# gotaku6629/CTC

Measured on AMD Instinct MI355X. Metric: ctc_samples_per_sec, higher is better.
Workload: dtype f32; 1 GPU; NoBlankCTC B=256 T=150 C=158 S<=20 fp32 (BASELINE configs[1]); variant=noblank, per_gpu_batch=256, global_batch=256, T=150, C=158, S=20, parallelism=dp1 (batch-sharded), launch=graph, graph_steps=50, step=fused loss+grad launch + scale_grad launch (loss.backward(), grad_out=1)

## Files before the change

### ctc_amd/build.py

```python
import os
import shutil
import subprocess
import sys

HERE = os.path.dirname(os.path.abspath(__file__))
CSRC = os.path.join(HERE, "csrc")
LIBDIR = os.path.join(HERE, "lib")
SO = os.path.join(LIBDIR, "libctc_amd.so")
SOURCES = ["api.hip", "noblank.hip", "binary.hip", "blank.hip", "decode.hip", "blank_align.hip", "targets.hip", "producer.hip"]
FLAGS = ["--offload-arch=gfx950", "-O3", "-std=c++17", "-fPIC", "-Wall", "-Wno-unused-function"]


def _hipcc():
    exe = shutil.which("hipcc") or "/opt/rocm/bin/hipcc"
    if not os.path.exists(exe):
        raise RuntimeError("hipcc not found: cannot build libctc_amd.so")
    return exe


def _stale():
    if not os.path.exists(SO):
        return True
    t = os.path.getmtime(SO)
    deps = [os.path.join(CSRC, f) for f in os.listdir(CSRC)] + \
           [os.path.join(HERE, "..", "include", "ctc_amd.h")]
    return any(os.path.getmtime(d) > t for d in deps)


def build(force=False, verbose=False, extra_flags=(), name=None):
    so = SO if name is None else os.path.join(LIBDIR, "libctc_amd_%s.so" % name)
    if name is None and any(f.startswith(("-DCTC_X_", "-DCTC_AMD_EXPERIMENTS", "-DCTC_AMD_FAULT_INJECT",
                                          "-DCTC_AMD_DIAGNOSTICS")) for f in extra_flags):
        raise RuntimeError("ctc_amd.build: experiment / diagnostics / fault-injection flags %s are refused for the "
                           "product library -- give the variant a name" % (list(extra_flags),))
    if name is None and not force and not _stale():
        return so
    os.makedirs(LIBDIR, exist_ok=True)
    objdir = os.path.join(LIBDIR, "obj" if name is None else "obj_" + name)
    os.makedirs(objdir, exist_ok=True)
    hipcc = _hipcc()
    procs = []
    for src in SOURCES:
        obj = os.path.join(objdir, src.replace(".hip", ".o"))
        cmd = [hipcc, *FLAGS, *extra_flags, "-c", os.path.join(CSRC, src), "-o", obj]
        if verbose:
            print(" ".join(cmd))
        procs.append((src, obj, subprocess.Popen(cmd, stdout=subprocess.PIPE, stderr=subprocess.STDOUT)))
    objs = []
    for src, obj, pr in procs:
        out, _ = pr.communicate()
        if pr.returncode != 0:
            raise RuntimeError("hipcc failed on %s:\n%s" % (src, out.decode()))
        if verbose and out:
            print(out.decode())
        objs.append(obj)
    subprocess.check_call([hipcc, "--offload-arch=gfx950", "-shared", "-fPIC", "-o", so + ".tmp", *objs])
    os.replace(so + ".tmp", so)
    return so


def _build_variant(name, flag, verbose):
    so = os.path.join(LIBDIR, "libctc_amd_%s.so" % name)
    if os.path.exists(so) and os.path.getmtime(so) >= os.path.getmtime(build()):
        return so
    return build(force=True, verbose=verbose, extra_flags=(flag,), name=name)


def build_diag(verbose=False):
    return _build_variant("diag", "-DCTC_AMD_DIAGNOSTICS", verbose)


def build_fault(verbose=False):
    return _build_variant("fault", "-DCTC_AMD_FAULT_INJECT", verbose)


def build_occupant():
    src = os.path.join(HERE, "..", "tools", "micro", "coresident.hip")
    so = os.path.join(LIBDIR, "libcoresident.so")
    if os.path.exists(so) and os.path.getmtime(so) >= os.path.getmtime(src):
        return so
    os.makedirs(LIBDIR, exist_ok=True)
    subprocess.check_call([_hipcc(), "--offload-arch=gfx950", "-O2", "-shared", "-fPIC", src, "-o", so + ".tmp"])
    os.replace(so + ".tmp", so)
    return so


HOST_EXT_DIR = os.path.join(LIBDIR, "ext")
HOST_EXT_SO = os.path.join(HOST_EXT_DIR, "ctc_amd_autograd_ext.so")


HOST_EXT_STAMP = os.path.join(HOST_EXT_DIR, "built_for_torch.txt")


def host_ext_is_current():
    import torch
    src = os.path.join(CSRC, "autograd_ext.cpp")
    if not (os.path.exists(HOST_EXT_SO) and os.path.exists(HOST_EXT_STAMP)):
        return False
    if os.path.getmtime(HOST_EXT_SO) < os.path.getmtime(src):
        return False
    return open(HOST_EXT_STAMP).read().strip() == torch.__version__


def build_host_ext(verbose=False):
    import torch
    src = os.path.join(CSRC, "autograd_ext.cpp")
    if host_ext_is_current():
        return HOST_EXT_SO
    from torch.utils import cpp_extension
    os.makedirs(HOST_EXT_DIR, exist_ok=True)
    cpp_extension.load(name="ctc_amd_autograd_ext", sources=[src], build_directory=HOST_EXT_DIR, extra_cflags=["-O2"],
                       with_cuda=False, verbose=verbose, is_python_module=False)
    with open(HOST_EXT_STAMP, "w") as f:
        f.write(torch.__version__)
    return HOST_EXT_SO


if __name__ == "__main__":
    if "--diag" in sys.argv:
        print(build_diag(verbose=True))
    else:
        print(build(force="--force" in sys.argv, verbose=True))
```

### ctc_amd/csrc/common.hpp

```cpp
#pragma once
#include <hip/hip_runtime.h>
#include <stdint.h>

#if !defined(CTC_AMD_EXPERIMENTS) &&                                                                            \
    (defined(CTC_X_NOSTATUS) || defined(CTC_X_NOREDUCE) || defined(CTC_X_NORETURN) || defined(CTC_X_NOCHAIN) || \
     defined(CTC_X_NOPRIO) || defined(CTC_X_NOREAD) || defined(CTC_X_NOWRITE) ||                                 \
     defined(CTC_X_WMASK) || defined(CTC_X_NOPROG) || defined(CTC_X_NORENORM) ||                                \
     defined(CTC_X_ROWDPP) || defined(CTC_X_SCALAR_STEP) || defined(CTC_X_NO_POOL_GATHER) || defined(CTC_X_FLOW_NO_GPRIO) || defined(CTC_X_FLOW_NOEXP) || defined(CTC_X_FLOW_NO_DELEGATE) || defined(CTC_X_FLOW_DELEGATE_OWN) || \
     defined(CTC_FLOW_TILE_WAVES))
#error "CTC_X_* experiment switches need -DCTC_AMD_EXPERIMENTS (A/B builds only, never the product library)"
#endif

namespace ctc {

constexpr int kWave = 64;
constexpr float kNeg = -10000000000000.0f;
constexpr float kInfeasible = 1.0e12f;

struct LaneStates { int K, SP; };
inline LaneStates lane_states(int S)
{
    int K = 1;
    while (K <= 4 && S > kWave * K) K *= 2;
    return {K, (S + K - 1) / K * K};
// ... 187 lines not shown
__device__ __forceinline__ float half_pick(float v, bool upper)
{
    const float lo = __builtin_bit_cast(float, __builtin_amdgcn_readlane(__builtin_bit_cast(int, v), 31));
    const float hi = __builtin_bit_cast(float, __builtin_amdgcn_readlane(__builtin_bit_cast(int, v), 63));
    return upper ? hi : lo;
}
__device__ __forceinline__ void halves_sum2(float &a, float &b, bool upper)
{
    asm volatile(CTC_REDUCE2_HALVES("v_add_f32_dpp") : "+v"(a), "+v"(b));
    a = half_pick(a, upper); b = half_pick(b, upper);
}
__device__ __forceinline__ void halves_max2(float &a, float &b, bool upper)
{
    asm volatile(CTC_REDUCE2_HALVES("v_max_f32_dpp") : "+v"(a), "+v"(b));
    a = half_pick(a, upper); b = half_pick(b, upper);
}

template <bool MAX>
__device__ __forceinline__ float group_reduce(float v, int G)
{
    v = MAX ? row16_max(v) : row16_sum(v);
    if (G >= 32) { const float o = __shfl_xor(v, 16, kWave); v = MAX ? fmaxf(v, o) : v + o; }
    if (G >= 64) { const float o = __shfl_xor(v, 32, kWave); v = MAX ? fmaxf(v, o) : v + o; }
    return v;
}

__device__ __forceinline__ float vmax(float a, float b)
{
    float r;
    asm("v_max_f32_e32 %0, %1, %2" : "=v"(r) : "v"(a), "v"(b));
    return r;
}

__device__ __forceinline__ float vmax3(float a, float b, float c)
{
    float r;
    asm("v_max3_f32 %0, %1, %2, %3" : "=v"(r) : "v"(a), "v"(b), "v"(c));
    return r;
}

constexpr float kLog2e = 1.4426950408889634f, kLn2 = 0.6931471805599453f;
__device__ __forceinline__ float fast_exp(float x) { return __builtin_amdgcn_exp2f(x * kLog2e); }
__device__ __forceinline__ float fast_log(float x) { return __builtin_amdgcn_logf(x) * kLn2; }

__device__ __forceinline__ float lse2(float a, float b)
{
    const float m = a > b ? a : b;
    const float t = __builtin_amdgcn_exp2f(-fabsf(a - b) * kLog2e);
    return __builtin_fmaf(__builtin_amdgcn_logf(1.0f + t), kLn2, m);
}

__device__ __forceinline__ int load_label(const void *p, int is64, int64_t i)
{
    return static_cast<const int32_t *>(p)[is64 ? 2 * i : i];
}

struct ScalarLengths {
    int64_t a, b;
    __device__ __forceinline__ ScalarLengths() : a(0), b(0) {}
    __device__ __forceinline__ ScalarLengths(const int64_t *pa, const int64_t *pb)
    {
        typedef const __attribute__((address_space(4))) int64_t const_i64;
        a = *(const_i64 *)(uintptr_t)pa;
        b = *(const_i64 *)(uintptr_t)pb;
    }
    __device__ __forceinline__ void get(int64_t &va, int64_t &vb) const
    {
        va = a;
        vb = b;
    }
};

__device__ __forceinline__ void bce_logs(float x, float &p, float &lp, float &lq)
{
    p = 1.0f / (1.0f + expf(-x));
    lp = fmaxf(logf(p), -100.0f);
    lq = fmaxf(logf(1.0f - p), -100.0f);
}

template <typename P>
__device__ __forceinline__ void stamp(const P &p, int slot)
{
    if (CTC_DIAG(p) >= 0 || CTC_DIAG(p) <= -100) return;
    if (blockIdx.x == 0 && wave_id() == -CTC_DIAG(p) - 1 && lane_id() == 0) {
        unsigned long long *o = reinterpret_cast<unsigned long long *>(p.counter) + 8 + 2 * slot;
        o[0] = __builtin_amdgcn_s_memtime();
        o[1] = __builtin_amdgcn_s_memrealtime();
    }
}

template <typename P>
__device__ __forceinline__ void stamp_setup(const P &p, int slot)
{
    if (CTC_DIAG(p) > -100 || CTC_DIAG(p) <= -200) return;
    if (blockIdx.x == 0 && wave_id() == -CTC_DIAG(p) - 100 && lane_id() == 0) {
        unsigned long long *o = reinterpret_cast<unsigned long long *>(p.counter) + 8 + 2 * slot;
        o[0] = __builtin_amdgcn_s_memtime();
        o[1] = __builtin_amdgcn_s_memrealtime();
    }
}

template <typename P>
__device__ __forceinline__ void stamp_mode(const P &p, int base, int slot)
{
    if (CTC_DIAG(p) > base || CTC_DIAG(p) <= base - 64) return;
    if (blockIdx.x == 0 && wave_id() == base - CTC_DIAG(p) && lane_id() == 0) {
        unsigned long long *o = reinterpret_cast<unsigned long long *>(p.counter) + 8 + 2 * (slot % 12);
        o[0] = __builtin_amdgcn_s_memtime();
        o[1] = __builtin_amdgcn_s_memrealtime();
    }
}

__device__ __forceinline__ void publish_value(float value, int b, float *nll)
{
    if (lane_id() == 0) __hip_atomic_store(&nll[b], value, __ATOMIC_RELAXED, __HIP_MEMORY_SCOPE_AGENT);
}
template <typename F>
__device__ __forceinline__ void ticket_and_reduce(int B, float *nll, float *loss, float loss_scale, unsigned *counter,
                                                  F per_sample)
{
    int last = 0;
    if (lane_id() == 0) {
        asm volatile("s_waitcnt vmcnt(0)" ::: "memory");
        unsigned ticket = __hip_atomic_fetch_add(counter, 1u, __ATOMIC_RELAXED, __HIP_MEMORY_SCOPE_AGENT);
        last = (ticket == (unsigned)(B - 1));
    }
    last = __builtin_amdgcn_readfirstlane(last);
    if (!last) return;
    float s = 0.f;
    for (int i = lane_id(); i < B; i += kWave)
        s += per_sample(__hip_atomic_load(&nll[i], __ATOMIC_RELAXED, __HIP_MEMORY_SCOPE_AGENT), i);
    s = wave_sum(s);
    if (lane_id() == 0) {
        loss[0] = s * loss_scale;
        __hip_atomic_store(counter, 0u, __ATOMIC_RELAXED, __HIP_MEMORY_SCOPE_AGENT);
        reset_arrivals(counter);
    }
}
template <typename F>
__device__ __forceinline__ void publish_and_reduce(float value, int b, int B, float *nll,
                                                   float *loss, float loss_scale,
                                                   unsigned *counter, F per_sample)
{
    publish_value(value, b, nll);
#ifndef CTC_X_NOREDUCE
    ticket_and_reduce(B, nll, loss, loss_scale, counter, per_sample);
#endif
}

constexpr int kAccIntBits = 13, kAccMaxB = 4095, kAccShards = 16;
__device__ __forceinline__ int acc_frac_bits(int B)
{
    return 40 - kAccIntBits - (B <= 1 ? 0 : 32 - __builtin_clz((unsigned)(B - 1)));
}
__host__ __device__ inline size_t acc_list_bytes(int B) { return 256 + (((size_t)4 * B + 255) & ~(size_t)255); }
__device__ __forceinline__ void publish_and_reduce_sum(float value, int b, int B, float *nll, float *loss,
                                                       float loss_scale, unsigned *counter)
{
    if (B > kAccMaxB) {
        publish_and_reduce(value, b, B, nll, loss, loss_scale, counter, [](float x, int) { return x; });
        return;
    }
    if (lane_id() != 0) return;
    unsigned long long *top = reinterpret_cast<unsigned long long *>(counter + 4);
    unsigned long long *shards = reinterpret_cast<unsigned long long *>(counter + 64);
    unsigned *nlist = counter + 6, *list = counter + 128;
    __hip_atomic_store(&nll[b], value, __ATOMIC_RELAXED, __HIP_MEMORY_SCOPE_AGENT);
// ... 38 lines not shown
```

### ctc_amd/csrc/noblank.hip

```cpp
#include <type_traits>

#include "lattice.hpp"
#include "launch.hpp"

namespace ctc {

struct NoblankParams {
    const float *x;
    int64_t st, sb;
    const void *lab;
    int lab64;
    const int64_t *in_len, *tgt_len;
    int T, B, C, S, SP;
    int stop;
    float loss_scale, grad_scale;
    float *nll, *loss, *grad;
    float *gamma;
    float *lattice;
    int64_t slab;
    unsigned *counter;
    int next_round;
    float ls_a, ls_b;
    int koff;
};
// ... 304 lines not shown
            const int t0 = base + w * kRows;
            for (int r = 0; r < kRows; r += per)
                if (t0 + r < Tlive)
                    posterior_row<true>(sm.al, sm.be, sm.em, sm.nxt, sm.dup, t0 + r + sub,
                                  r + sub < kRows && t0 + r + sub < Tlive, L, p.SP, G);
            if (CTC_DIAG(p) == 4) continue;
            stamp(p, 6);
            if (base == 0) {
                rows.grad(p, sm, b, t0, Tlive, first);
            } else {
                Rows<CHR> extra;
                extra.load(p, b, t0, Tlive);
                extra.grad(p, sm, b, t0, Tlive, first);
            }
        }
    } else {
        rows_grad_generic(p, sm, b, Tlive, L);
    }
    stamp(p, 7);
}

}

#include "noblank_pipe.hpp"
#include "noblank_xr.hpp"
#include "noblank_r16.hpp"
#ifdef CTC_AMD_DIAGNOSTICS
#include "noblank_km.hpp"
#endif

namespace ctc {

__global__ __launch_bounds__(256) void scale_grad_kernel(float *g, const float *go, size_t n)
{
    const float s = *go;
    if (s == 1.0f) return;
    const size_t stride = (size_t)gridDim.x * blockDim.x;
    size_t i = (size_t)blockIdx.x * blockDim.x + threadIdx.x;
    if ((reinterpret_cast<uintptr_t>(g) & 15) == 0) {
        float4 *g4 = reinterpret_cast<float4 *>(g);
        const size_t n4 = n / 4;
        for (size_t k = i; k < n4; k += stride) {
            float4 v = g4[k];
            v.x *= s; v.y *= s; v.z *= s; v.w *= s;
            g4[k] = v;
        }
        for (size_t k = n4 * 4 + i; k < n; k += stride) g[k] *= s;
    } else {
        for (size_t k = i; k < n; k += stride) g[k] *= s;
    }
}

template <typename E>
__global__ __launch_bounds__(256) void scale_grad_lowp_kernel(E *g, const float *go, size_t n)
{
    const float s = *go;
    if (s == 1.0f) return;
    const size_t stride = (size_t)gridDim.x * blockDim.x;
    const size_t i = (size_t)blockIdx.x * blockDim.x + threadIdx.x;
    size_t done = 0;
    if ((reinterpret_cast<uintptr_t>(g) & 7) == 0) {
        wt_u2 *g4 = reinterpret_cast<wt_u2 *>(g);
        const size_t n4 = n / 4;
        const f2_t s2 = {s, s};
        for (size_t k = i; k < n4; k += stride) {
            wt_u2 v = g4[k];
            v.x = r16_narrow2<E>(r16_widen2<E>(v.x) * s2);
            v.y = r16_narrow2<E>(r16_widen2<E>(v.y) * s2);
            g4[k] = v;
        }
        done = n4 * 4;
    }
    for (size_t k = done + i; k < n; k += stride) g[k] = (E)((float)g[k] * s);
}


struct NoblankSwitches {
    bool no_pipe, no_xr, no_r16, no_ps, km;
    bool nograd;
    int stop;
};
static const NoblankSwitches &noblank_switches()
{
    static const NoblankSwitches sw = {diag_env("CTC_AMD_NOPIPE") != 0, diag_env("CTC_AMD_NOXR") != 0,
                                       diag_env("CTC_AMD_NOR16") != 0,  diag_env("CTC_AMD_NOPS") != 0,
                                       diag_env("CTC_AMD_KM") != 0,     diag_env("CTC_AMD_DEBUG_NOGRAD") != 0,
                                       diag_env("CTC_AMD_DEBUG_STOP")};
    return sw;
}

static int noblank_params(NoblankParams &p, const void *x, int64_t stride_t, int64_t stride_b,
                          const void *labels, int labels_i64, const int64_t *in_len, const int64_t *tgt_len,
                          int T, int B, int C, int S, float loss_scale, float grad_scale,
                          float *nll, float *loss, void *grad, float *gamma, void *workspace, float label_smoothing,
                          const NoblankSwitches &sw)
{
    if (!x || !labels || !in_len || !tgt_len || !nll || !(loss || gamma) || !workspace) return CTC_AMD_ERR_BAD_ARGUMENT;
    if (T < 1 || B < 1 || C < 1 || S < 1) return CTC_AMD_ERR_BAD_ARGUMENT;
    const NoblankSizes z = noblank_sizes(T, C, S);
    char *ws = static_cast<char *>(workspace);
    p.x = static_cast<const float *>(x); p.st = stride_t; p.sb = stride_b;
    p.lab = labels; p.lab64 = labels_i64;
    p.in_len = in_len; p.tgt_len = tgt_len;
    p.T = T; p.B = B; p.C = C; p.S = S; p.SP = z.SP;
    p.stop = sw.stop;
    p.loss_scale = loss_scale; p.grad_scale = grad_scale;
    p.nll = nll; p.loss = gamma ? reinterpret_cast<float *>(ws + 32) : loss;
    p.grad = sw.nograd ? nullptr : static_cast<float *>(grad);
    p.gamma = gamma;
    p.counter = static_cast<unsigned *>(workspace);
    p.lattice = z.glb ? reinterpret_cast<float *>(ws + 256 + acc_list_bytes(B)) : nullptr;
    p.slab = z.glb ? (int64_t)noblank_lattice_floats(T, z.SP) : 0;
    p.next_round = 0; p.koff = 0;
    const bool smooth = label_smoothing >= 0.f;
    p.ls_b = smooth ? (1.f - label_smoothing) / (float)C : 0.f;
    p.ls_a = smooth ? label_smoothing - p.ls_b : 1.f;
    return 0;
}

struct NoblankQuery {
    int T, B, C, S;
    int dtype;
    int64_t st, sb;
    unsigned x_low, grad_low;
    bool want_grad, want_gamma, smooth;
    int cus;
    NoblankSwitches sw;
};
enum NoblankFamily { kNoblankUnsupported = 0, kNoblankR16, kNoblankKm, kNoblankXr, kNoblankPipelined, kNoblankFused };
struct NoblankPlan {
    int family;
    int n4, n2, nt, ps;
    int ch, dual;
    int K, glb;
    int grid;
    size_t lds;
    int next_round, koff;
};

static bool r16_takes(const NoblankQuery &q, const NoblankSizes &z, unsigned align, int &n4, int &n2)
{
    return z.K == 1 && q.T <= kPipeMaxT && q.C % 2 == 0 && q.st % 2 == 0 && q.sb % 2 == 0 && q.x_low % align == 0 &&
           q.grad_low % align == 0 && r16_shape(q.C, n4, n2) && z.SP <= 31 && r16_smem_bytes(q.T, z.SP, q.C) <= kMaxLds;
}

static NoblankPlan noblank_plan(const NoblankQuery &q)
{
    const NoblankSizes z = noblank_sizes(q.T, q.C, q.S);
    NoblankPlan pl = {};
    if (z.K > 4) return pl;
    const bool lowp = q.dtype != CTC_AMD_F32;
    const int esz = lowp ? 2 : 4, cus = q.cus;
    pl.grid = q.B;
    int n4 = 0, n2 = 0;
    const bool r16 = r16_takes(q, z, lowp ? 4 : 8, n4, n2);
    const bool r16_only = q.smooth || lowp;
    const bool fast = z.K == 1 && q.C <= 256 && q.T <= kPipeMaxT && !q.sw.no_pipe && !z.glb && !q.want_gamma;
    if (r16 && (q.want_gamma || lowp || (fast && !q.sw.no_r16))) {
        pl.n4 = n4; pl.n2 = n2;
        pl.lds = r16_smem_bytes(q.T, z.SP, q.C);
        if (q.want_gamma) { pl.family = kNoblankR16; return pl; }
        pl.nt = (size_t)2 * esz * q.T * q.B * q.C > ((size_t)230 << 20);
#ifdef CTC_AMD_DIAGNOSTICS
        const int koff = km_offset(q.T, q.S);
        if (q.sw.km && !lowp && km_smem_bytes(q.T, z.SP, q.C) <= kMaxLds && koff >= 0) {
            pl.family = kNoblankKm;
            pl.lds = km_smem_bytes(q.T, z.SP, q.C);
            pl.koff = koff;
            pl.next_round = (q.B > cus && (size_t)q.T * ((q.C * 4 + 127) / 128) <= (size_t)kKmWorkers * kWave) ? cus : 0;
            return pl;
        }
#endif
        pl.family = kNoblankR16;
        pl.next_round = (q.B > cus && (size_t)q.T * ((q.C * esz + 127) / 128) <= (size_t)kPipeWorkers * kWave) ? cus : 0;
        pl.ps = q.B > 2 * cus && cus > 0 && !q.sw.no_ps && q.want_grad && 4 * n4 + 2 * n2 <= 12;
        if (pl.ps) pl.grid = cus;
        return pl;
    }
    if (r16_only || (z.glb && z.smem > kMaxLds)) return NoblankPlan{};
    if (fast) {
        pl.ch = (q.C + kWave - 1) / kWave;
        pl.dual = q.B > cus && 2 * z.smem <= kMaxLds;
        const size_t xsmem = xr_smem_bytes(q.T, z.SP, q.C);
        const bool xr = !q.sw.no_xr && xsmem <= kMaxLds && (!pl.dual || 2 * xsmem <= kMaxLds);
        pl.family = xr ? kNoblankXr : kNoblankPipelined;
        pl.lds = xr ? xsmem : z.smem;
        return pl;
    }
    pl.family = kNoblankFused;
    pl.K = z.K; pl.glb = z.glb;
    pl.ch = q.C <= 256 && !z.glb ? (q.C + kWave - 1) / kWave : 0;
    pl.lds = z.smem;
    return pl;
}

template <int N, int... Ns, typename F>
static int with_constant(int n, F f)
{
    if constexpr (sizeof...(Ns) == 0) {
        return f(std::integral_constant<int, N>());
    } else {
        return n == N ? f(std::integral_constant<int, N>()) : with_constant<Ns...>(n, f);
    }
}
template <typename F>
static int with_row_chunks(int n4, int n2, F f)
{
    return with_constant<1, 2, 4, 5, 6, 8, 9, 10, 12, 13, 14, 16>(4 * n4 + n2, [&](auto k) {
        return f(std::integral_constant<int, decltype(k)::value / 4>(), std::integral_constant<int, decltype(k)::value % 4>());
    });
}

static int noblank_launch(const NoblankPlan &pl, int dtype, NoblankParams &p, hipStream_t s)
{
    const dim3 grid(pl.grid), block(kThreads);
    p.next_round = pl.next_round; p.koff = pl.koff;
    switch (pl.family) {
        case kNoblankR16:
            return with_row_chunks(pl.n4, pl.n2, [&](auto n4, auto n2) {
                return with_constant<0, 1>(pl.nt, [&](auto nt) {
                    return with_constant<CTC_AMD_BF16, CTC_AMD_F16, CTC_AMD_F32>(dtype, [&](auto dt) {
                        using E = std::conditional_t<decltype(dt)::value == CTC_AMD_BF16, __bf16,
                                                     std::conditional_t<decltype(dt)::value == CTC_AMD_F16, _Float16, float>>;
                        constexpr int A = decltype(n4)::value, Bq = decltype(n2)::value;
                        constexpr bool NT = decltype(nt)::value != 0;
                        if constexpr (4 * A + 2 * Bq <= 12)
                            if (pl.ps) return launch<noblank_r16_kernel<A, Bq, NT, true, E>>(grid, block, pl.lds, s, p);
                        return launch<noblank_r16_kernel<A, Bq, NT, false, E>>(grid, block, pl.lds, s, p);
                    });
                });
            });
#ifdef CTC_AMD_DIAGNOSTICS
        case kNoblankKm:
            return with_row_chunks(pl.n4, pl.n2, [&](auto n4, auto n2) {
                return with_constant<0, 1>(pl.nt, [&](auto nt) {
                    return launch<noblank_km_kernel<decltype(n4)::value, decltype(n2)::value, decltype(nt)::value != 0>>(
                        grid, block, pl.lds, s, p);
                });
            });
#endif
        case kNoblankXr:
        case kNoblankPipelined:
            return with_constant<1, 2, 3, 4>(pl.ch, [&](auto ch) {
                return with_constant<0, 1>(pl.dual, [&](auto dual) {
                    constexpr int CH = decltype(ch)::value;
                    constexpr bool DUAL = decltype(dual)::value != 0;
                    return pl.family == kNoblankXr ? launch<noblank_xr_kernel<CH, DUAL>>(grid, block, pl.lds, s, p)
                                                   : launch<noblank_pipelined_kernel<CH, DUAL>>(grid, block, pl.lds, s, p);
                });
            });
        case kNoblankFused:
            return with_constant<1, 2, 4>(pl.K, [&](auto k) {
                constexpr int K = decltype(k)::value;
                if (pl.glb) return launch<noblank_fused_kernel<K, 0, true>>(grid, block, pl.lds, s, p);
                return with_constant<1, 2, 3, 4, 0>(pl.ch, [&](auto ch) {
                    return launch<noblank_fused_kernel<K, decltype(ch)::value>>(grid, block, pl.lds, s, p);
                });
            });
        default: return CTC_AMD_ERR_UNSUPPORTED_SHAPE;
    }
}

static int noblank_run(const void *x, int64_t stride_t, int64_t stride_b,
                       const void *labels, int labels_i64,
                       const int64_t *in_len, const int64_t *tgt_len,
                       int T, int B, int C, int S,
                       float loss_scale, float grad_scale,
                       float *nll, float *loss, void *grad,
                       void *workspace, void *stream, float label_smoothing, int x_dtype = CTC_AMD_F32,
                       float *gamma = nullptr)
{
    const NoblankSwitches sw = gamma ? NoblankSwitches{} : noblank_switches();
    NoblankParams p;
    if (const int rc = noblank_params(p, x, stride_t, stride_b, labels, labels_i64, in_len, tgt_len, T, B, C, S, loss_scale,
                                      grad_scale, nll, loss, grad, gamma, workspace, label_smoothing, sw))
        return rc;
    const NoblankQuery q = {T, B, C, S, x_dtype, stride_t, stride_b,
                            (unsigned)(reinterpret_cast<uintptr_t>(x) & 15), (unsigned)(reinterpret_cast<uintptr_t>(grad) & 15),
                            p.grad != nullptr, gamma != nullptr, label_smoothing >= 0.f,
                            device_cus(),
                            sw};
    return noblank_launch(noblank_plan(q), x_dtype, p, static_cast<hipStream_t>(stream));
}

static dim3 scale_grad_grid(size_t n)
{
    size_t blocks = (n / 4 + 255) / 256;
    static const int cap = diag_env("CTC_AMD_SCALE_BLOCKS", 1024);
    if (blocks > (size_t)cap) blocks = cap;
    if (blocks < 1) blocks = 1;
    return dim3((unsigned)blocks);
}

}

using namespace ctc;

extern "C" int ctc_amd_noblank_loss_grad(const float *x, int64_t stride_t, int64_t stride_b,
                                         const void *labels, int labels_i64,
                                         const int64_t *in_len, const int64_t *tgt_len,
                                         int T, int B, int C, int S,
                                         float loss_scale, float grad_scale,
                                         float *nll, float *loss, float *grad,
                                         void *workspace, void *stream)
{
    return noblank_run(x, stride_t, stride_b, labels, labels_i64, in_len, tgt_len, T, B, C, S, loss_scale, grad_scale,
                       nll, loss, grad, workspace, stream, -1.f);
}

extern "C" int ctc_amd_noblank_smoothed_loss_grad(const float *x, int64_t stride_t, int64_t stride_b,
                                                  const void *labels, int labels_i64,
// ... 90 lines not shown
```

### ctc_amd/csrc/noblank_r16.hpp

```cpp
#pragma once

namespace ctc {

typedef float f2_t __attribute__((ext_vector_type(2)));

#define CTC_ROW16(OP)                                                                   \
    "s_nop 1\n\t" OP " %0, %0, %0 quad_perm:[1,0,3,2] row_mask:0xf bank_mask:0xf\n\t"   \
    "s_nop 1\n\t" OP " %0, %0, %0 quad_perm:[2,3,0,1] row_mask:0xf bank_mask:0xf\n\t"   \
    "s_nop 1\n\t" OP " %0, %0, %0 row_half_mirror row_mask:0xf bank_mask:0xf\n\t"       \
    "s_nop 1\n\t" OP " %0, %0, %0 row_mirror row_mask:0xf bank_mask:0xf\n\t"            \
    "s_nop 1"
__device__ __forceinline__ void row16_allmax(float &v) { asm volatile(CTC_ROW16("v_max_f32_dpp") : "+v"(v)); }
__device__ __forceinline__ void row16_allsum(float &v) { asm volatile(CTC_ROW16("v_add_f32_dpp") : "+v"(v)); }
__device__ __forceinline__ void row16_allmax(int &v) { asm volatile(CTC_ROW16("v_max_i32_dpp") : "+v"(v)); }

constexpr int kR16Pad = 2 * kPrefetch + 1;
#ifndef CTC_R16_BLOCK
#define CTC_R16_BLOCK 16
#endif
constexpr int kR16Block = CTC_R16_BLOCK;
__host__ __device__ inline int r16_pitch(int T)
{
    int tp = T + 2 * kR16Pad + 1;
    while ((tp & 3) != 2) ++tp;
    return tp;
}

__device__ __forceinline__ int r16_row(int T, int u, int g, int k)
{
    const int H = (T + 1) >> 1, idx = 2 * kPipeWorkers * g + 2 * u + (k >> 1);
    if ((k & 1) == 0) return idx < H ? idx : -1;
    return idx < T - H ? T - 1 - idx : -1;
}

struct R16Smem {
    int TP;
    cell_t *em, *al, *be;
    float *dummy, *stage, *cs;
    int *cnt, *lab, *occ, *done;
    __device__ R16Smem(float *base, int T, int SP, int RP)
    {
        TP = r16_pitch(T);
        cell_t *lat = reinterpret_cast<cell_t *>(base);
        em = lat + kR16Pad;
        al = em + (size_t)(SP + 1) * TP;
        be = al + (size_t)(SP + 1) * TP;
        dummy = reinterpret_cast<float *>(lat + (size_t)3 * (SP + 1) * TP);
        cnt = reinterpret_cast<int *>(dummy + 8);
        lab = cnt + 16;
        occ = lab + ((SP + 3) & ~3);
        cs = reinterpret_cast<float *>(occ + ((SP + 3) & ~3) + 4);
        done = reinterpret_cast<int *>(cs + 4 * kPipeWorkers);
        stage = cs + 64;
    }
};

static size_t r16_smem_bytes(int T, int SP, int C)
{
    const int RP = 32 * ((C + 31) / 32);
    return (size_t)3 * (SP + 1) * r16_pitch(T) * 8 + (8 + 16 + 2 * ((SP + 3) & ~3) + 4 + 64) * 4 +
           (size_t)kPipeWorkers * 4 * RP * 4;
}

template <bool FWD>
__device__ __forceinline__ cell_t r16_chain(const NoblankParams &p, const R16Smem &sm, int T, int Tb, int L, int SP, const int lane)
{
    constexpr int G = kPipeRows / 4;
    constexpr int D = FWD ? 1 : -1;
    const int lrow = lane < SP ? lane : SP;
    const cell_t *erow = sm.em + (size_t)lrow * sm.TP;
    cell_t *orow = (FWD ? sm.al : sm.be) + (size_t)lrow * sm.TP;
    typedef float pair_t __attribute__((ext_vector_type(4)));
    float m;
    int k;

    const int H = (T + 1) >> 1;
    const int pos0 = FWD ? 0 : T - Tb;
    const int own = FWD ? H : T - H;
    typedef const volatile __attribute__((address_space(3))) int lds_cvint;
    const int *cp = sm.cnt + (lane < kPipeWorkers ? lane : 0);
    int have = 0;
    bool starved = false;
    auto wait_upto = [&](int i_last) {
        const int q = pos0 + (i_last < Tb ? i_last : Tb - 1);
        int ng = q / (2 * kPipeWorkers) + 1;
        if (q >= own || ng > G) ng = G;
        if (ng <= have) return;
        const int need = lane < kPipeWorkers ? 4 * ng : 0;
        int spins = 0;
        while (__builtin_amdgcn_ballot_w64(*(lds_cvint *)cp < need) != 0) {
            if (++spins >= kSpinLimit) { starved = true; break; }
            __builtin_amdgcn_s_sleep(1);
        }
        lds_order();
        have = ng;
    };
#define CTC_R16_STEP_ASM(K, M, EM, EK, K2, T2, DPP)                                                  \
            "v_max_i32_dpp %[kk], " K ", " K " " DPP "\n\t"                                           \
            "v_add_u32 " K2 ", %[kk], " EK "\n\t"                                                     \
            "v_sub_u32 %[d1], " K ", %[kk]\n\t"                                                       \
            "v_sub_u32_dpp %[d2], " K ", %[kk] " DPP "\n\t"                                           \
            "v_ldexp_f32 %[d1], " EM ", %[d1]\n\t"                                                    \
            "v_ldexp_f32 %[d2], " EM ", %[d2]\n\t"                                                    \
// ... 296 lines not shown
        for (int k = 0; k < N2; ++k) o2[k] = *reinterpret_cast<const f2_t *>(trow + off2(k, i16));
#pragma unroll
        for (int j = 0; j < N4; ++j) {
            const f4_t o = o4[j];
            f2_t olo = {o.x, o.y}, ohi = {o.z, o.w};
            if (LS) { olo += cb2; ohi += cb2; }
            const f2_t xlo = {a[j].x, a[j].y}, xhi = {a[j].z, a[j].w};
            const f2_t vlo = __builtin_elementwise_fma(xlo, r2, olo), vhi = __builtin_elementwise_fma(xhi, r2, ohi);
            if (!(kLast4 && j == N4 - 1) || col_ok) {
                if constexpr (kLowp) {
                    const wt_u2 n = {r16_narrow2<E>(vlo), r16_narrow2<E>(vhi)};
                    grad_store<NT, wt_u2, 4>(reinterpret_cast<wt_u2 *>(g + off4(j, i16)), n);
                } else {
                    const f4_t v = {vlo.x, vlo.y, vhi.x, vhi.y};
                    grad_store<NT>(reinterpret_cast<f4_t *>(g + off4(j, i16)), v);
                }
            }
        }
#pragma unroll
        for (int k = 0; k < N2; ++k) {
            f2_t o = o2[k];
            if (LS) o += cb2;
            const f2_t v = __builtin_elementwise_fma(c[k], r2, o);
            if (k < N2 - 1 || col_ok) {
                if constexpr (kLowp) grad_store<NT, unsigned, 4>(reinterpret_cast<unsigned *>(g + off2(k, i16)), r16_narrow2<E>(v));
                else grad_store<NT>(reinterpret_cast<f2_t *>(g + off2(k, i16)), v);
            }
        }
    }
    __device__ __forceinline__ void touch() const
    {
        if constexpr (kLowp) {
#pragma unroll
            for (int j = 0; j < N4; ++j) asm volatile("" ::"v"(this->ra[j]));
#pragma unroll
            for (int k = 0; k < N2; ++k) asm volatile("" ::"v"(this->rc[k]));
        } else {
#pragma unroll
            for (int j = 0; j < N4; ++j) asm volatile("" ::"v"(a[j]));
#pragma unroll
            for (int k = 0; k < N2; ++k) asm volatile("" ::"v"(c[k]));
        }
    }
    template <bool NT>
    __device__ static __forceinline__ void store_zero(E *g, int i16, bool col_ok)
    {
        if constexpr (kLowp) {
            const wt_u2 z4 = {0u, 0u};
#pragma unroll
            for (int j = 0; j < N4; ++j)
                if (!(kLast4 && j == N4 - 1) || col_ok) grad_store<NT, wt_u2, 4>(reinterpret_cast<wt_u2 *>(g + off4(j, i16)), z4);
#pragma unroll
            for (int k = 0; k < N2; ++k)
                if (k < N2 - 1 || col_ok) grad_store<NT, unsigned, 4>(reinterpret_cast<unsigned *>(g + off2(k, i16)), 0u);
            return;
        }
        const f4_t z4 = {0.f, 0.f, 0.f, 0.f};
        const f2_t z2 = {0.f, 0.f};
#pragma unroll
        for (int j = 0; j < N4; ++j)
            if (!(kLast4 && j == N4 - 1) || col_ok) grad_store<NT>(reinterpret_cast<f4_t *>(g + off4(j, i16)), z4);
#pragma unroll
        for (int k = 0; k < N2; ++k)
            if (k < N2 - 1 || col_ok) grad_store<NT>(reinterpret_cast<f2_t *>(g + off2(k, i16)), z2);
    }
};

static bool r16_shape(int C, int &n4, int &n2)
{
    if (C < 2 || C > 256 || (C & 1)) return false;
    const int U = (C + 31) / 32;
    if (U & 1) { n4 = U / 2; n2 = 1; }
    else if ((C & 3) == 0) { n4 = U / 2; n2 = 0; }
    else { n4 = U / 2 - 1; n2 = 2; }
    return true;
}

template <typename E>
__device__ __forceinline__ const E *r16_xrow(const NoblankParams &p, int t, int b)
{
    return reinterpret_cast<const E *>(p.x) + (int64_t)t * p.st + (int64_t)b * p.sb;
}
template <int N4, int N2, bool NT, bool PS = false, typename E = float>
__global__ __launch_bounds__(kThreads, 4) void noblank_r16_kernel(NoblankParams p)
{
    extern __shared__ float4 smem_raw[];
    typedef R16Row<N4, N2, E> Row;
    constexpr int RP = Row::kCols;
    constexpr int G = kPipeRows / 4;
    const R16Smem sm(reinterpret_cast<float *>(smem_raw), p.T, p.SP, RP);
    const int tid = threadIdx.x, w = wave_id(), lane = lane_id();
    int vb = blockIdx.x;
    int b = xcd_sample(vb, p.B);
    if (tid == 64 * kChainB) note_arrival(p.counter, b);
    const int u = (w == 0 || w == kChainB) ? -1 : (w < kChainB ? w - 1 : w - 2);
    const int rho = lane >> 4, i16 = lane & 15;

    if (CTC_DIAG(p) == 1) return;
    stamp(p, 0);
    stamp_setup(p, 0);
    auto spread = [&](int which) {
        if (CTC_DIAG(p) != -50 || w != 1 || lane != 0) return;
        const int bid = blockIdx.x, nb = gridDim.x;
        const int slot = bid == 0 ? 0 : bid == nb / 2 ? 2 : bid == nb - 1 ? 4 : -1;
        if (slot < 0) return;
        unsigned long long *o = reinterpret_cast<unsigned long long *>(p.counter) + 8 + 2 * (slot + which);
        o[0] = __builtin_amdgcn_s_memtime();
        o[1] = __builtin_amdgcn_s_memrealtime();
    };
    spread(0);
    ScalarLengths len(p.in_len + b, p.tgt_len + b);
    int tv0[G];
    Row v[G];
#ifdef CTC_R16_NX
    constexpr int NX = PS ? CTC_R16_NX : 0;
#else
    constexpr int NX = PS ? (NT ? 2 : 3) : 0;
#endif
    Row nx[NX > 0 ? NX : 1];
    const bool col_ok = Row::off_last(i16) < p.C;
    const int c_last = col_ok ? Row::off_last(i16) : p.C - (Row::kLast4 ? 4 : 2);
    const int Hh = (p.T + 1) >> 1;
    bool grp[G];
#pragma unroll
    for (int g = 0; g < G; ++g) grp[g] = u >= 0 && 2 * kPipeWorkers * g + 2 * u < Hh;
    int klab = 0;
    if (PS && w == 0 && lane < p.S) klab = load_label(p.lab, p.lab64, (int64_t)b * p.S + lane);
    if (u >= 0) {
#pragma unroll
        for (int g = 0; g < G; ++g) {
            tv0[g] = r16_row(p.T, u, g, rho);
            if (g >= NX) v[g].load(r16_xrow<E>(p, tv0[g] >= 0 ? tv0[g] : 0, b), i16, c_last);
            else nx[g].load(r16_xrow<E>(p, tv0[g] >= 0 ? tv0[g] : 0, b), i16, c_last);
        }
        stamp_setup(p, 1);
        if (PS) {
#pragma unroll
            for (int g = 0; g < G; ++g) {
                if (g < NX) nx[g].touch();
                else v[g].touch();
            }
        }
    }
    const float ninf = -__builtin_inff();
    typedef const volatile __attribute__((address_space(3))) int lds_cvint;
    int Tb = 0, L = 0, bn = b, vbn = vb, klab_n = 0;
    bool more = false;
    ScalarLengths len_n;
    const cell_t zero = make_cell(0.f, 0);
    auto begin = [&](const bool chain_role) -> bool {
        int64_t Tb64, L64;
        len.get(Tb64, L64);
        stamp_setup(p, 2);
        const bool ok = L64 >= 1 && L64 <= p.S && Tb64 >= L64 && Tb64 <= p.T;
        Tb = ok ? (int)Tb64 : 0;
        L = ok ? (int)L64 : 0;
        vbn = vb + (int)gridDim.x;
        more = PS && vbn < p.B;
        bn = more ? xcd_sample(vbn, p.B) : b;
        if (PS) len_n = ScalarLengths(p.in_len + bn, p.tgt_len + bn);
        klab_n = 0;
        if (chain_role && w == 0) {
            int k = 0;
            if (lane < L) {
                k = (PS ? klab : load_label(p.lab, p.lab64, (int64_t)b * p.S + lane)) % p.C;
                if (k < 0) k += p.C;
            }
            if (lane < p.SP) sm.lab[lane] = k;
            if (more && lane < p.S) klab_n = load_label(p.lab, p.lab64, (int64_t)bn * p.S + lane);
        }
        stamp_setup(p, 3);
        for (int i = tid; i < (p.SP + 1) * sm.TP; i += kThreads) sm.em[i - kR16Pad] = zero;
        if (tid < 16) sm.cnt[tid] = 0;
        if (tid == 16) *sm.done = 0;
        if (tid == 17) sm.occ[((p.SP + 3) & ~3) + 1] = 0;
        if (tid < 8) sm.dummy[tid] = 0.f;
        stamp_setup(p, 4);
        asm volatile("s_waitcnt lgkmcnt(0)\n\ts_barrier" ::: "memory");
        stamp(p, 1);
        stamp_setup(p, 5);
        stamp_mode(p, -200, (vb - (int)blockIdx.x) / (int)gridDim.x);
        if ((vb - (int)blockIdx.x) / (int)gridDim.x < 6) stamp_mode(p, -400, (vb - (int)blockIdx.x) / (int)gridDim.x);
        return CTC_DIAG(p) != 2;
    };
    auto advance = [&]() -> bool {
        stamp_mode(p, -300, (vb - (int)blockIdx.x) / (int)gridDim.x);
        if ((vb - (int)blockIdx.x) / (int)gridDim.x < 6) stamp_mode(p, -400, 6 + (vb - (int)blockIdx.x) / (int)gridDim.x);
        if (!more) return false;
        vb = vbn;
        b = bn;
        len = len_n;
        klab = klab_n;
        asm volatile("s_waitcnt lgkmcnt(0)\n\ts_barrier" ::: "memory");
        return true;
    };
    auto chain_sample = [&](const NoblankParams &p, const int lane) {
    const R16Smem sm(reinterpret_cast<float *>(smem_raw), p.T, p.SP, RP);
    if (Tb == 0) {
        if (w == 0)
            publish_and_reduce_sum(-kNeg, b, p.B, p.nll, p.loss, p.loss_scale, p.counter);
        return;
    }
    {
        __builtin_amdgcn_s_setprio(3);
        if (w == 0) {
            const cell_t a = r16_chain<true>(p, sm, p.T, Tb, L, p.SP, lane);
            stamp(p, 11);
            bool late = false;
            {
                int spins = 0;
                while (*(lds_cvint *)sm.done < kPipeWorkers) {
                    if (++spins >= kSpinLimit) { late = true; break; }
                    __builtin_amdgcn_s_sleep(2);
                }
                lds_order();
            }
            const float csum = wave_sum(lane < 4 * kPipeWorkers ? sm.cs[lane] : 0.f);
            const float am = a.x;
            float nll = am > 0.f ? -(__builtin_amdgcn_logf(am) + (float)(cell_k(a) - kXrBias) + csum) * kLn2 : -kNeg;
            if (am != am) nll = am;
            if (late) {
                raise_status(p.counter, kStatusNoblankStarved);
                nll = __builtin_nanf("");
            }
            publish_and_reduce_sum(nll, b, p.B, p.nll, p.loss, p.loss_scale, p.counter);
            if (CTC_DIAG(p) == -50 && lane == 0) {
                const int bid = blockIdx.x, nb = gridDim.x;
                const int slot = bid == 0 ? 6 : bid == nb / 2 ? 7 : bid == nb - 1 ? 8 : -1;
                if (slot >= 0) {
                    unsigned long long *o = reinterpret_cast<unsigned long long *>(p.counter) + 8 + 2 * slot;
                    o[0] = __builtin_amdgcn_s_memtime();
                    o[1] = __builtin_amdgcn_s_memrealtime();
                }
            }
        } else if (p.grad || p.gamma) {
            r16_chain<false>(p, sm, p.T, Tb, L, p.SP, lane);
            stamp(p, 11);
        }
    }
    };

    auto worker_sample = [&](const NoblankParams &p, const int lane, const int u) {
    const R16Smem sm(reinterpret_cast<float *>(smem_raw), p.T, p.SP, RP);
    const int rho = lane >> 4, i16 = lane & 15;
    int tv[G];
#pragma unroll
    for (int g = 0; g < G; ++g) tv[g] = PS ? opaque_v(tv0[g]) : tv0[g];
    const bool has_grad = PS || p.grad != nullptr, has_gamma = !PS && !Row::kLowp && p.gamma != nullptr;
    auto load_next = [&]() {
        if (!PS) return;
#pragma unroll
        for (int g = 0; g < NX; ++g) nx[g].load(r16_xrow<E>(p, tv[g] >= 0 ? tv[g] : 0, bn), i16, c_last);
    };
#define CTC_R16_RELOAD(g)                                                                             \
    do {                                                                                              \
        if (PS && (g) >= NX) v[g].load(r16_xrow<E>(p, tv[g] >= 0 ? tv[g] : 0, bn), i16, c_last); \
    } while (0)
    if (!PS && Tb == 0) {
        if (p.grad) {
#pragma unroll
            for (int g = 0; g < G; ++g)
                if (tv[g] >= 0) Row::template store_zero<NT>(reinterpret_cast<E *>(p.grad) + ((int64_t)tv[g] * p.B + b) * p.C, i16, col_ok);
        }
        if (!Row::kLowp && p.gamma) {
#pragma unroll
            for (int g = 0; g < G; ++g)
                for (int l = i16; l < p.S && tv[g] >= 0; l += 16) p.gamma[((int64_t)b * p.T + tv[g]) * p.S + l] = 0.f;
        }
        return;
    }
    float *tile = sm.stage + (size_t)u * 4 * RP;
    float *trow = tile + rho * RP;
    int lst[2];
    float *gat[2];
#pragma unroll
    for (int s = 0; s < 2; ++s) {
        lst[s] = 16 * s + i16;
        gat[s] = trow + (lst[s] < p.SP ? sm.lab[lst[s]] : 0);
    }
    const bool own[2] = {lst[0] < L, lst[1] < L};
    const bool smooth = p.ls_b != 0.f;
    cell_t *const spare_w = reinterpret_cast<cell_t *>(sm.dummy);
    float mrow[G];
#pragma unroll
    for (int g = 0; g < G; ++g) {
        if (g == 0) __builtin_amdgcn_s_setprio(2);
        else __builtin_amdgcn_s_setprio(1);
        if (g < NX) v[g] = nx[g];
        if (grp[g]) {
            Row &x = v[g];
            x.widen();
            const int t = tv[g];
            const bool live = t >= 0 && t < Tb;
            float m = x.max();
            row16_allmax(m);
            mrow[g] = m;
            if (CTC_DIAG(p) < 0 && g == 0) stamp(p, 6);
            x.to_tile(trow, i16);
            lds_order();
            float xv[2];
#pragma unroll
            for (int s = 0; s < 2; ++s) xv[s] = *gat[s];
            lds_order();
#pragma unroll
            for (int s = 0; s < 2; ++s) {
                const float ec = (xv[s] - m) * kLog2e;
                const float e2 = fmaxf(smooth ? p.ls_a * ec : ec, kXrMinLog2);
                const float fl = __builtin_floorf(e2);
                const float pm = __builtin_amdgcn_exp2f(e2 - fl);
                cell_t *dst = (live && lst[s] < p.SP) ? sm.em + lst[s] * sm.TP + t : spare_w;
                *dst = own[s] ? make_cell(pm, (int)fl) : zero;
            }
            lds_order();
        } else {
            mrow[g] = 0.f;
        }
        sm.cnt[u] = 4 * (g + 1);
        __builtin_amdgcn_sched_barrier(0);
        if (CTC_DIAG(p) < 0) stamp(p, 8 + g);
    }
    __builtin_amdgcn_s_setprio(0);
    load_next();
    float rs[G];
    float cacc = 0.f;
#pragma unroll
    for (int g = 0; g < G; ++g) {
        rs[g] = 0.f;
        if (!grp[g]) continue;
        Row &x = v[g];
        const int t = tv[g];
        const bool live = t >= 0 && t < Tb;
        const float m = mrow[g];
        float sx = 0.f;
        if (smooth) {
            sx = x.sum(col_ok);
            row16_allsum(sx);
        }
        const float mb = -m * kLog2e;
        float sum = x.exp_sum(mb, col_ok ? mb : ninf);
        row16_allsum(sum);
        const float l2sum = __builtin_amdgcn_logf(sum);
        rs[g] = live ? p.grad_scale * __builtin_amdgcn_rcpf(sum) : 0.f;
        const float cst = smooth ? __builtin_fmaf(p.ls_b, __builtin_fmaf(sx - (float)p.C * m, kLog2e, -(float)p.C * l2sum), -p.ls_a * l2sum)
                                 : -l2sum;
        cacc += live ? cst : 0.f;
    }
    if (i16 == 0) sm.cs[4 * u + rho] = cacc;
    lds_order();
    if (lane == 0) __hip_atomic_fetch_add(sm.done, 1, __ATOMIC_RELAXED, __HIP_MEMORY_SCOPE_WORKGROUP);
    stamp(p, 2);
    if (u == kPipeWorkers - 1 && has_grad) {
        const int kl = lane < p.SP ? sm.lab[lane] : -1;
        int oc = 0;
        for (int l2 = 0; l2 < L; ++l2) {
            const int q = __builtin_amdgcn_readlane(kl, l2);
            oc += (l2 < lane && q == kl) ? 1 : 0;
        }
        if (lane >= L) oc = 0;
        int mo = 0;
        while (__builtin_amdgcn_ballot_w64(oc > mo) != 0) ++mo;
        if (lane < p.SP) sm.occ[lane] = oc;
        sm.occ[(p.SP + 3) & ~3] = mo;
        lds_order();
        sm.occ[((p.SP + 3) & ~3) + 1] = 1;
    }
    float prefetched = 0.f;
    if (!PS && p.next_round > 0 && (int)blockIdx.x + p.next_round < p.B) {
        const int nb = xcd_sample(blockIdx.x + p.next_round, p.B);
        const int line = u * kWave + lane;
        const int lines_per_row = (p.C * (int)sizeof(E) + 127) / 128;
        const int t = line / lines_per_row, c = (line - t * lines_per_row) * (128 / (int)sizeof(E));
// ... 208 lines not shown
```

Baseline: 19.37 million samples/s.

## Preload kernel args and defer tail row loads in noblank r16 kernel

Passes the hot scalar parameters (x pointer, strides, T, B, C) as separate leading kernel arguments and compiles noblank.hip with kernarg preload of 9 SGPRs, so they are available without a kernarg memory load at wave start. In the non-PS path the last rows' logit loads are deferred until after the first row is touched, and setup work (LDS struct, arrival note, length loads, group mask) is moved after the initial loads are issued. The aim is to shorten kernel prologue latency and spread memory traffic, at the cost of scheduling barriers and a larger argument list. The diagnostics stamp logic is also extended to select blocks.

```diff
diff --git a/ctc_amd/build.py b/ctc_amd/build.py
--- a/ctc_amd/build.py
+++ b/ctc_amd/build.py
@@ -9,6 +9,7 @@
 SO = os.path.join(LIBDIR, "libctc_amd.so")
 SOURCES = ["api.hip", "noblank.hip", "binary.hip", "blank.hip", "decode.hip", "blank_align.hip", "targets.hip", "producer.hip"]
 FLAGS = ["--offload-arch=gfx950", "-O3", "-std=c++17", "-fPIC", "-Wall", "-Wno-unused-function"]
+SOURCE_FLAGS = {"noblank.hip": ["-mllvm", "-amdgpu-kernarg-preload-count=9"]}
 
 
 def _hipcc():
@@ -42,7 +43,7 @@
     procs = []
     for src in SOURCES:
         obj = os.path.join(objdir, src.replace(".hip", ".o"))
-        cmd = [hipcc, *FLAGS, *extra_flags, "-c", os.path.join(CSRC, src), "-o", obj]
+        cmd = [hipcc, *FLAGS, *SOURCE_FLAGS.get(src, ()), *extra_flags, "-c", os.path.join(CSRC, src), "-o", obj]
         if verbose:
             print(" ".join(cmd))
         procs.append((src, obj, subprocess.Popen(cmd, stdout=subprocess.PIPE, stderr=subprocess.STDOUT)))
diff --git a/ctc_amd/csrc/common.hpp b/ctc_amd/csrc/common.hpp
--- a/ctc_amd/csrc/common.hpp
+++ b/ctc_amd/csrc/common.hpp
@@ -293,7 +293,10 @@
 __device__ __forceinline__ void stamp(const P &p, int slot)
 {
     if (CTC_DIAG(p) >= 0 || CTC_DIAG(p) <= -100) return;
-    if (blockIdx.x == 0 && wave_id() == -CTC_DIAG(p) - 1 && lane_id() == 0) {
+    const int d = -CTC_DIAG(p) - 1, sel = d >> 4;
+    if (sel > 2) return;
+    const int bid = sel == 0 ? 0 : sel == 1 ? (int)gridDim.x / 2 : (int)gridDim.x - 1;
+    if ((int)blockIdx.x == bid && wave_id() == (d & 15) && lane_id() == 0) {
         unsigned long long *o = reinterpret_cast<unsigned long long *>(p.counter) + 8 + 2 * slot;
         o[0] = __builtin_amdgcn_s_memtime();
         o[1] = __builtin_amdgcn_s_memrealtime();
diff --git a/ctc_amd/csrc/noblank.hip b/ctc_amd/csrc/noblank.hip
--- a/ctc_amd/csrc/noblank.hip
+++ b/ctc_amd/csrc/noblank.hip
@@ -410,10 +410,13 @@
 };
 static const NoblankSwitches &noblank_switches()
 {
-    static const NoblankSwitches sw = {diag_env("CTC_AMD_NOPIPE") != 0, diag_env("CTC_AMD_NOXR") != 0,
-                                       diag_env("CTC_AMD_NOR16") != 0,  diag_env("CTC_AMD_NOPS") != 0,
-                                       diag_env("CTC_AMD_KM") != 0,     diag_env("CTC_AMD_DEBUG_NOGRAD") != 0,
-                                       diag_env("CTC_AMD_DEBUG_STOP")};
+    static NoblankSwitches sw = {diag_env("CTC_AMD_NOPIPE") != 0, diag_env("CTC_AMD_NOXR") != 0,
+                                 diag_env("CTC_AMD_NOR16") != 0,  diag_env("CTC_AMD_NOPS") != 0,
+                                 diag_env("CTC_AMD_KM") != 0,     diag_env("CTC_AMD_DEBUG_NOGRAD") != 0,
+                                 diag_env("CTC_AMD_DEBUG_STOP")};
+#ifdef CTC_AMD_DIAGNOSTICS
+    sw.stop = diag_env("CTC_AMD_DEBUG_STOP");
+#endif
     return sw;
 }
 
@@ -539,6 +542,12 @@
     });
 }
 
+template <auto kern>
+static int r16_launch(dim3 grid, dim3 block, size_t lds, hipStream_t s, const NoblankParams &p)
+{
+    return launch<kern>(grid, block, lds, s, p.x, p.st, p.sb, p.T, p.B, p.C, p);
+}
+
 static int noblank_launch(const NoblankPlan &pl, int dtype, NoblankParams &p, hipStream_t s)
 {
     const dim3 grid(pl.grid), block(kThreads);
@@ -553,8 +562,8 @@
                         constexpr int A = decltype(n4)::value, Bq = decltype(n2)::value;
                         constexpr bool NT = decltype(nt)::value != 0;
                         if constexpr (4 * A + 2 * Bq <= 12)
-                            if (pl.ps) return launch<noblank_r16_kernel<A, Bq, NT, true, E>>(grid, block, pl.lds, s, p);
-                        return launch<noblank_r16_kernel<A, Bq, NT, false, E>>(grid, block, pl.lds, s, p);
+                            if (pl.ps) return r16_launch<noblank_r16_kernel<A, Bq, NT, true, E>>(grid, block, pl.lds, s, p);
+                        return r16_launch<noblank_r16_kernel<A, Bq, NT, false, E>>(grid, block, pl.lds, s, p);
                     });
                 });
             });
diff --git a/ctc_amd/csrc/noblank_r16.hpp b/ctc_amd/csrc/noblank_r16.hpp
--- a/ctc_amd/csrc/noblank_r16.hpp
+++ b/ctc_amd/csrc/noblank_r16.hpp
@@ -19,6 +19,10 @@
 #define CTC_R16_BLOCK 16
 #endif
 constexpr int kR16Block = CTC_R16_BLOCK;
+#ifndef CTC_R16_DEFER
+#define CTC_R16_DEFER 2
+#endif
+constexpr int kR16Deferred = CTC_R16_DEFER;
 __host__ __device__ inline int r16_pitch(int T)
 {
     int tp = T + 2 * kR16Pad + 1;
@@ -481,17 +485,17 @@
     return reinterpret_cast<const E *>(p.x) + (int64_t)t * p.st + (int64_t)b * p.sb;
 }
 template <int N4, int N2, bool NT, bool PS = false, typename E = float>
-__global__ __launch_bounds__(kThreads, 4) void noblank_r16_kernel(NoblankParams p)
+__global__ __launch_bounds__(kThreads, 4) void noblank_r16_kernel(const float *x_, int64_t st_, int64_t sb_, int T_, int B_, int C_,
+                                                                  NoblankParams p)
 {
+    p.x = x_; p.st = st_; p.sb = sb_; p.T = T_; p.B = B_; p.C = C_;
     extern __shared__ float4 smem_raw[];
     typedef R16Row<N4, N2, E> Row;
     constexpr int RP = Row::kCols;
     constexpr int G = kPipeRows / 4;
-    const R16Smem sm(reinterpret_cast<float *>(smem_raw), p.T, p.SP, RP);
     const int tid = threadIdx.x, w = wave_id(), lane = lane_id();
     int vb = blockIdx.x;
     int b = xcd_sample(vb, p.B);
-    if (tid == 64 * kChainB) note_arrival(p.counter, b);
     const int u = (w == 0 || w == kChainB) ? -1 : (w < kChainB ? w - 1 : w - 2);
     const int rho = lane >> 4, i16 = lane & 15;
 
@@ -508,7 +512,6 @@
         o[1] = __builtin_amdgcn_s_memrealtime();
     };
     spread(0);
-    ScalarLengths len(p.in_len + b, p.tgt_len + b);
     int tv0[G];
     Row v[G];
 #ifdef CTC_R16_NX
@@ -517,21 +520,21 @@
     constexpr int NX = PS ? (NT ? 2 : 3) : 0;
 #endif
     Row nx[NX > 0 ? NX : 1];
+    constexpr int NE = PS ? G : (G - kR16Deferred > 0 ? G - kR16Deferred : 1);
     const bool col_ok = Row::off_last(i16) < p.C;
     const int c_last = col_ok ? Row::off_last(i16) : p.C - (Row::kLast4 ? 4 : 2);
-    const int Hh = (p.T + 1) >> 1;
-    bool grp[G];
-#pragma unroll
-    for (int g = 0; g < G; ++g) grp[g] = u >= 0 && 2 * kPipeWorkers * g + 2 * u < Hh;
     int klab = 0;
     if (PS && w == 0 && lane < p.S) klab = load_label(p.lab, p.lab64, (int64_t)b * p.S + lane);
     if (u >= 0) {
 #pragma unroll
-        for (int g = 0; g < G; ++g) {
+        for (int g = 0; g < NE; ++g) {
             tv0[g] = r16_row(p.T, u, g, rho);
             if (g >= NX) v[g].load(r16_xrow<E>(p, tv0[g] >= 0 ? tv0[g] : 0, b), i16, c_last);
             else nx[g].load(r16_xrow<E>(p, tv0[g] >= 0 ? tv0[g] : 0, b), i16, c_last);
         }
+        __builtin_amdgcn_sched_barrier(0);
+#pragma unroll
+        for (int g = NE; g < G; ++g) tv0[g] = r16_row(p.T, u, g, rho);
         stamp_setup(p, 1);
         if (PS) {
 #pragma unroll
@@ -541,6 +544,13 @@
             }
         }
     }
+    const R16Smem sm(reinterpret_cast<float *>(smem_raw), p.T, p.SP, RP);
+    if (tid == 64 * kChainB) note_arrival(p.counter, b);
+    ScalarLengths len(p.in_len + b, p.tgt_len + b);
+    const int Hh = (p.T + 1) >> 1;
+    bool grp[G];
+#pragma unroll
+    for (int g = 0; g < G; ++g) grp[g] = u >= 0 && 2 * kPipeWorkers * g + 2 * u < Hh;
     const float ninf = -__builtin_inff();
     typedef const volatile __attribute__((address_space(3))) int lds_cvint;
     int Tb = 0, L = 0, bn = b, vbn = vb, klab_n = 0;
@@ -686,6 +696,13 @@
         if (g == 0) __builtin_amdgcn_s_setprio(2);
         else __builtin_amdgcn_s_setprio(1);
         if (g < NX) v[g] = nx[g];
+        if (!PS && g == 0 && NE < G) {
+            if (grp[0]) v[0].touch();
+            __builtin_amdgcn_sched_barrier(0);
+#pragma unroll
+            for (int h = NE; h < G; ++h) v[h].load(r16_xrow<E>(p, tv[h] >= 0 ? tv[h] : 0, b), i16, c_last);
+            __builtin_amdgcn_sched_barrier(0);
+        }
         if (grp[g]) {
             Row &x = v[g];
             x.widen();
```

Measured after the change: 19.46 million samples/s, median of 5. No clear change (+0.5%).
